# yuxng/PoseCNN

Hardware: NVIDIA H100
Metric: frames/sec on 640x480 RGB, 21 classes, batch 32 (VGG16 + Hough + ROI pose head) (higher is better)
Workload: dtype bf16 operands / fp32 accumulate (conv stack, 1x1 heads), fp16 operands / fp32 accumulate (fc6-fc8), fp32 / int32 elsewhere

## Files before the change

### include/posecnn_b200.h

```cpp
#ifndef POSECNN_B200_H_
#define POSECNN_B200_H_

#include <stddef.h>
#include <stdint.h>

#ifdef __cplusplus
extern "C" {
#endif

#define PCNN_OK 0
#define PCNN_E_INVALID (-1)
#define PCNN_E_WORKSPACE (-2)
#define PCNN_E_CUDA (-3)

#define PCNN_MAX_ROI 128
#define PCNN_HOUGH_MAX_ROWS (PCNN_MAX_ROI * 9)

const char* pcnn_last_error(void);
int pcnn_version(void);

int pcnn_hough_vote_workspace_bytes(int B, int H, int W, int C, int skip_pixels, float threshold_vote,
                                    size_t* bytes);
int pcnn_hough_vote_fwd(const int32_t* label, const float* vertex, const float* extents, const float* meta,
                        const float* gt, int B, int H, int W, int C, int num_gt, int num_meta, int is_train,
                        float inlier_threshold, int label_threshold, float threshold_vote,
                        float threshold_percentage, int skip_pixels, float* top_box, float* top_pose,
                        float* top_target, float* top_weight, int32_t* top_domain, int32_t* num_rois,
                        int32_t* status, void* workspace, size_t workspace_bytes, void* stream);
int pcnn_hough_vote_fwd_ex(const int32_t* label, const float* vertex, const float* lowres, const float* bias_vertex,
                           const float* extents, const float* meta, const float* gt, int B, int batch_global,
                           int batch_offset, int H, int W, int C, int num_gt, int num_meta, int is_train,
                           float inlier_threshold, int label_threshold, float threshold_vote,
                           float threshold_percentage, int skip_pixels, float* top_box, float* top_pose,
                           float* top_target, float* top_weight, int32_t* top_domain, int32_t* num_rois,
                           int32_t* status, void* workspace, size_t workspace_bytes, void* stream);
int pcnn_hough_vote_planes(const int32_t* label, const float* vertex, const float* extents, const float* meta,
                           int B, int H, int W, int C, int num_meta, float inlier_threshold,
                           int label_threshold, int skip_pixels, float* votes, void* workspace,
                           size_t workspace_bytes, void* stream);
int pcnn_hough_vote_bwd(float* grad_label, float* grad_vertex, int B, int H, int W, int C, void* stream);

int pcnn_roi_pool_fwd(const float* bottom, const float* rois, int num_rois, int channel_rois, int batch,
                      int height, int width, int channels, int pooled_height, int pooled_width,
                      float spatial_scale, int pool_channel, float* top, int32_t* argmax, void* stream);
int pcnn_roi_pool_fwd_bf16(const void* bottom_bf16, const float* rois, int num_rois, int channel_rois, int batch,
                           int height, int width, int channels, int pooled_height, int pooled_width,
                           float spatial_scale, float* top, int32_t* argmax, void* stream);
int pcnn_roi_pool_bwd(const float* top_diff, const int32_t* argmax, const float* rois, int batch, int num_rois,
                      int channel_rois, int height, int width, int channels, int pooled_height,
                      int pooled_width, float spatial_scale, int pool_channel, float* bottom_diff,
                      void* stream);

int pcnn_hard_label_fwd(const float* prob, const int32_t* gt, int B, int H, int W, int C, float threshold,
                        float* top, void* stream);
int pcnn_hard_label_bwd(int B, int H, int W, int C, float* grad_prob, float* grad_gt, void* stream);

int pcnn_backproject_fwd(const float* data, const float* label, const float* depth, const float* meta,
                         const float* label_3d, int B, int H, int W, int Cf, int C, int num_meta,
                         int grid_size, int kernel_size, float threshold, float* top_data, float* top_label,
                         float* top_flag, void* stream);
int pcnn_backproject_bwd(const float* top_diff, const float* depth, const float* meta, int B, int H, int W,
                         int Cf, int num_meta, int grid_size, float* bottom_diff, void* stream);

int pcnn_project_fwd(const float* data, const float* depth, const float* meta, int B, int H, int W, int Cf,
                     int num_meta, int grid_size, float* top, void* stream);
int pcnn_project_bwd(const float* top_diff, const float* depth, const float* meta, int B, int H, int W, int Cf,
                     int num_meta, int grid_size, int kernel_size, float threshold, float* bottom_diff,
                     void* stream);

int pcnn_average_distance_workspace_bytes(int N, size_t* bytes);
int pcnn_average_distance_fwd(const float* prediction, const float* target, const float* weight,
                              const float* point, const float* symmetry, int N, int C, int P, float margin,
                              float* loss, float* bottom_diff, void* workspace, size_t workspace_bytes,
                              void* stream);
int pcnn_average_distance_bwd(const float* top_diff, const float* bottom_diff, int N, int channels,
                              float* output, void* stream);

int pcnn_conv_bf16_tc(const void* in_bf16, const void* weights_bf16, const float* bias, void* out_bf16, int B,
                      int H, int W, int Cin, int Cout, int ksize, int relu, int block_n, void* stream);
int pcnn_conv_pool_bf16_tc(const void* in_bf16, const void* weights_bf16, const float* bias, void* out_pooled_bf16,
                           int B, int H, int W, int Cin, int Cout, int ksize, int relu, int block_n, void* stream);
int pcnn_conv3x3_small_cin(const float* in, const float* weights_hwio, const float* bias, void* out_bf16, int B,
                           int H, int W, int Cin, int Cout, int relu, void* stream);
int pcnn_im2col_c3(const void* in, int in_is_u8, const float* mean3_host, void* out_bf16, int B, int H, int W,
                   void* stream);
int pcnn_im2col_depth(const float* depth, const float* mean3_host, void* out_bf16, int B, int H, int W, void* stream);
int pcnn_conv1_fused_tc(const void* in, int in_is_u8, const float* mean3_host, const void* weights_bf16,
                        const float* bias, void* out_bf16, int B, int H, int W, int relu, void* stream);
int pcnn_conv1_depth_fused_tc(const float* depth, const float* mean3_host, const void* weights_bf16, const float* bias,
                              void* out_bf16, int B, int H, int W, int relu, void* stream);
int pcnn_maxpool2x2_bf16(const void* in_bf16, void* out_bf16, int B, int H, int W, int C, void* stream);

int pcnn_conv_wgrad_workspace_bytes(int B, int H, int W, int Cin, int Cout, int ksize, size_t* bytes);
int pcnn_conv_wgrad_bf16_tc(const void* x_bf16, const void* dz_bf16, int B, int H, int W, int Cin, int Cout, int ksize,
                            float scale, const float* w_f32, float decay, float* dW, void* workspace, size_t workspace_bytes,
                            void* stream);
int pcnn_fc_wgrad_f16_tc(const void* x_f16, const void* dy_f16, int rows, int Cin, int Cout, float scale, const float* w_f32,
                         float decay, float* dW, void* workspace, size_t workspace_bytes, void* stream);
int pcnn_bias_ws_bytes(int C, size_t* bytes);
int pcnn_relu_bwd_bf16(const void* g_bf16, const void* y_bf16, size_t npix, int C, int has_relu, void* dz_bf16, float scale,
                       const float* b, float decay, float* db, void* bias_ws, size_t bias_ws_bytes, void* stream);
int pcnn_maxpool_relu_bwd_bf16(const void* g_bf16, const void* y_bf16, int B, int H, int W, int C, void* dz_bf16, float scale,
                               const float* b, float decay, float* db, void* bias_ws, size_t bias_ws_bytes, void* stream);
int pcnn_add_to_bf16(const void* a_bf16, const void* b_bf16, const float* b_f32, size_t n, void* out_bf16, void* stream);

int pcnn_add_up2_bf16(const void* a4_bf16, const void* a5_bf16, int B, int h, int w, int C, void* out_bf16, void* stream);
int pcnn_up2_bwd_bf16(const void* dadd_bf16, const void* y5_bf16, int B, int h, int w, int C, void* d5_bf16, void* stream);
int pcnn_pack_lowres(const void* sc_bf16, int Cs, const void* vt_bf16, int Cv, int B, int h, int w, int C, float* lowres, void* stream);
int pcnn_up8_heads_bwd_ex(const float* prob, const float* score, const int32_t* gt, const float* cls_loss_out, float upstream_cls,
                          float threshold, const float* vertex_pred, const float* lowres, const float* bias_vertex, const float* centers,
                          const float* vertex_loss_out, float upstream_vertex, float w_inside, float sigma, int B, int h, int w, int C,
                          int Cs, int Cv, void* d_sc_bf16, void* d_vt_bf16, float* dbias, void* workspace, size_t workspace_bytes,
                          void* stream);
int pcnn_pose_chain_bwd(const float* bottom_diff, const float* poses_tanh, const float* poses_weight, int N, int D, float upstream,
                        void* dpre_f16, int ld, void* stream);
int pcnn_sgd_momentum(float* w, float* accum, const float* grad, size_t n, float lr, float mu, float wd, float gscale, void* copy16,
                      int kind, void* stream);
int pcnn_loss_cls_hard_raw_fwd(const float* score_raw, const float* prob, const int32_t* gt, int B, int H, int W, int C,
                               float threshold, float* loss_out, void* workspace, size_t workspace_bytes, void* stream);
int pcnn_fc_dgrad_f16_tc(const void* dy_f16, const void* w_in_out_f16, int M, int N, int K, const void* relu_mask_f16, void* out_f16,
                         int ld_out, void* workspace, size_t workspace_bytes, void* stream);
int pcnn_transpose16(const void* in, int rows, int cols, void* out, void* stream);
int pcnn_half_to_float(const void* src_f16, size_t n, float scale, float* dst, void* stream);

int pcnn_roi_pool_pair_f16(const void* f5_bf16, int H5, int W5, const void* f4_bf16, int H4, int W4, int C, int B,
                            int batch_offset, const float* rois, int num_rois, int roi_stride, int pooled_h,
                            int pooled_w, float scale5, float scale4, void* out_f16, void* stream);
int pcnn_fc_workspace_bytes(int M, int N, int K, size_t* bytes);
int pcnn_fc_f16_tc(const void* a_f16, const void* w_f16, const float* bias, int M, int N, int K, int n_valid, int act,
                   void* out_f16, int ld_out, float* out_f32, void* workspace, size_t workspace_bytes, void* stream);

int pcnn_domain_tail(const void* fc9_f16, int rows, int ld, const float* w10, const float* b10, const int32_t* label_domain,
                     float loss_scale, float grad_scale, float* domain_score, float* domain_prob, int32_t* domain_label,
                     float* loss, float* amax, float* dw10, float* db10, float* db9, void* dpre9_f16, void* stream);
int pcnn_domain_grad_merge(const void* a_f16, float scale_a, const void* b_f16, float scale_b, size_t n, float* dst, void* stream);

int pcnn_lowres_heads(const void* score4, const void* score5, const void* vert4, const void* vert5,
                      const float* w_score, const float* w_vertex, int B, int h, int w, int Cs, int Cv, int C,
                      float* lowres, void* stream);
int pcnn_up8_heads(const float* lowres, const float* bias_score, const float* bias_vertex, int B, int h, int w,
                   int C, int32_t* label, float* vertex, float* prob, float* score, void* stream);
int pcnn_deconv_bilinear(const float* in, float* out, int B, int h, int w, int C, int k, int s, void* stream);

int pcnn_nms_pose_fwd(const float* rois, const float* poses_init, const float* poses_pred, const int* num_rois_dev,
                      int num_rows, int capacity, int num_classes, float thresh, int per_image, int32_t* keep,
                      float* out_rois, float* out_poses, int32_t* num_keep, void* stream);

int pcnn_vertex_targets_instances_fwd(const int32_t* label, const int32_t* mask, const float* instances, int B, int H, int W,
                                      int C, int I, float w_inside, float* targets, float* weights, void* stream);
int pcnn_pack_pose_meta_fwd(const float* poses, const int32_t* cls, const float* intrinsics, int B, int I, float im_scale,
                            int flip_x, float* pose_blob, int32_t* num_rows, float* meta, void* stream);
int pcnn_train_loss_workspace_bytes(size_t* bytes);
int pcnn_vertex_targets_fwd(const int32_t* label, const float* centers, int B, int H, int W, int C, float w_inside,
                            float* targets, float* weights, void* stream);
int pcnn_loss_cls_hard_fwd(const float* score, const float* prob, const int32_t* gt, int B, int H, int W, int C,
                           float threshold, float* loss_out, float upstream, float* grad_score, void* workspace,
                           size_t workspace_bytes, void* stream);
int pcnn_smooth_l1_vertex_fwd(const float* pred, const float* targets, const float* weights, size_t n, float sigma,
                              float* loss_out, float upstream, float* grad_pred, void* workspace, size_t workspace_bytes,
                              void* stream);
int pcnn_vertex_loss_fused_fwd(const float* pred, const int32_t* label, const float* centers, int B, int H, int W, int C,
                               float w_inside, float sigma, float* loss_out, float upstream, float* grad_pred,
                               void* workspace, size_t workspace_bytes, void* stream);
int pcnn_vertex_loss_fused_lowres_fwd(const float* lowres, const float* bias_vertex, const int32_t* label, const float* centers, int B,
                                      int H, int W, int C, float w_inside, float sigma, float* loss_out, void* workspace,
                                      size_t workspace_bytes, void* stream);

#define PCNN_AUG_BACKGROUND 0
#define PCNN_AUG_CHROMATIC 1
#define PCNN_AUG_DH 2
#define PCNN_AUG_DL 3
#define PCNN_AUG_DS 4
#define PCNN_AUG_NOISE 5
// ... 15 lines not shown
```

### posecnn_b200/conv.py

```python
from __future__ import annotations

import torch

from ._lib import check, lib, ptr, stream


def hwio_to_tc(weights_hwio: torch.Tensor, dtype=torch.bfloat16) -> torch.Tensor:
    kh, kw, ci, co = weights_hwio.shape
    return weights_hwio.permute(3, 0, 1, 2).reshape(co, kh * kw * ci).to(dtype).contiguous()


def hwio_to_tc_dgrad(weights_hwio: torch.Tensor) -> torch.Tensor:
    kh, kw, ci, co = weights_hwio.shape
    flipped = torch.flip(weights_hwio, dims=(0, 1)).permute(0, 1, 3, 2).contiguous()
    return hwio_to_tc(flipped)


def conv_bf16(x: torch.Tensor, w_tc: torch.Tensor, bias: torch.Tensor, ksize: int, relu: bool, block_n: int = 0,
              out: torch.Tensor | None = None) -> torch.Tensor:
    assert x.is_cuda and x.dtype == torch.bfloat16 and x.is_contiguous() and x.dim() == 4
    assert w_tc.dtype == torch.bfloat16 and w_tc.is_contiguous() and bias.dtype == torch.float32
    B, H, W, Cin = x.shape
    Cout = w_tc.shape[0]
    assert w_tc.shape[1] == ksize * ksize * Cin
    if out is None:
        out = torch.empty((B, H, W, Cout), dtype=torch.bfloat16, device=x.device)
    check(lib().pcnn_conv_bf16_tc(ptr(x), ptr(w_tc), ptr(bias), ptr(out), B, H, W, Cin, Cout, int(ksize), int(bool(relu)),
                                  int(block_n), stream()))
    return out


def conv_pool_bf16(x: torch.Tensor, w_tc: torch.Tensor, bias: torch.Tensor, ksize: int, relu: bool, block_n: int = 0) -> torch.Tensor:
    assert x.is_cuda and x.dtype == torch.bfloat16 and x.is_contiguous() and x.dim() == 4
    B, H, W, Cin = x.shape
    Cout = w_tc.shape[0]
    out = torch.empty((B, H // 2, W // 2, Cout), dtype=torch.bfloat16, device=x.device)
    check(lib().pcnn_conv_pool_bf16_tc(ptr(x), ptr(w_tc), ptr(bias), ptr(out), B, H, W, Cin, Cout, int(ksize), int(bool(relu)),
                                       int(block_n), stream()))
    return out


def conv3x3_small_cin(x: torch.Tensor, w_hwio: torch.Tensor, bias: torch.Tensor, relu: bool = True) -> torch.Tensor:
    assert x.is_cuda and x.dtype == torch.float32 and x.is_contiguous()
    B, H, W, Cin = x.shape
    Cout = w_hwio.shape[3]
    out = torch.empty((B, H, W, Cout), dtype=torch.bfloat16, device=x.device)
    check(lib().pcnn_conv3x3_small_cin(ptr(x), ptr(w_hwio.contiguous()), ptr(bias), ptr(out), B, H, W, Cin, Cout,
                                       int(bool(relu)), stream()))
    return out


def maxpool2x2(x: torch.Tensor) -> torch.Tensor:
    assert x.is_cuda and x.dtype == torch.bfloat16 and x.is_contiguous()
    B, H, W, C = x.shape
    out = torch.empty((B, H // 2, W // 2, C), dtype=torch.bfloat16, device=x.device)
    check(lib().pcnn_maxpool2x2_bf16(ptr(x), ptr(out), B, H, W, C, stream()))
    return out


def im2col_c3(x: torch.Tensor, mean=None) -> torch.Tensor:
    import ctypes
    assert x.is_cuda and x.is_contiguous() and x.shape[3] == 3 and x.dtype in (torch.float32, torch.uint8)
    B, H, W, _ = x.shape
    out = torch.empty((B, H, W, 64), dtype=torch.bfloat16, device=x.device)
    m = (ctypes.c_float * 3)(*(mean if mean is not None else (0.0, 0.0, 0.0)))
    check(lib().pcnn_im2col_c3(ptr(x), int(x.dtype == torch.uint8), m, ptr(out), B, H, W, stream()))
    return out


def im2col_depth(depth: torch.Tensor, mean) -> torch.Tensor:
    import ctypes
    assert depth.is_cuda and depth.is_contiguous() and depth.dtype == torch.float32 and depth.dim() == 3
    B, H, W = depth.shape
    out = torch.empty((B, H, W, 64), dtype=torch.bfloat16, device=depth.device)
    m = (ctypes.c_float * 3)(*mean)
    check(lib().pcnn_im2col_depth(ptr(depth), m, ptr(out), B, H, W, stream()))
    return out


def conv1_1_weights_to_tc(w_hwio: torch.Tensor) -> torch.Tensor:
    co = w_hwio.shape[3]
    w = torch.zeros((co, 64), dtype=torch.float32, device=w_hwio.device)
    w[:, :27] = w_hwio.reshape(27, co).t()
    return w.to(torch.bfloat16).contiguous()


def conv1_fused(x: torch.Tensor, w_tc64: torch.Tensor, bias: torch.Tensor, mean=None, relu: bool = True) -> torch.Tensor:
    import ctypes
    assert x.is_cuda and x.is_contiguous() and x.shape[3] == 3 and x.dtype in (torch.float32, torch.uint8)
    assert w_tc64.shape == (64, 64) and w_tc64.dtype == torch.bfloat16
    B, H, W, _ = x.shape
    out = torch.empty((B, H, W, 64), dtype=torch.bfloat16, device=x.device)
    m = (ctypes.c_float * 3)(*(mean if mean is not None else (0.0, 0.0, 0.0)))
    check(lib().pcnn_conv1_fused_tc(ptr(x), int(x.dtype == torch.uint8), m, ptr(w_tc64), ptr(bias), ptr(out), B, H, W,
                                    int(bool(relu)), stream()))
    return out


def conv1_depth_fused(depth: torch.Tensor, w_tc64: torch.Tensor, bias: torch.Tensor, mean, relu: bool = True) -> torch.Tensor:
    import ctypes
    assert depth.is_cuda and depth.is_contiguous() and depth.dtype == torch.float32 and depth.dim() == 3
    B, H, W = depth.shape
    out = torch.empty((B, H, W, 64), dtype=torch.bfloat16, device=depth.device)
    m = (ctypes.c_float * 3)(*mean)
    check(lib().pcnn_conv1_depth_fused_tc(ptr(depth), m, ptr(w_tc64), ptr(bias), ptr(out), B, H, W, int(bool(relu)), stream()))
    return out
```

### posecnn_b200/csrc/conv_tc.cu

```cuda
#include <cuda.h>
#include <cuda_bf16.h>

#include <type_traits>

#include "common.cuh"
#include "tc_common.cuh"

namespace pcnn {
namespace convtc {

constexpr int kTileH = 8, kTileW = 16;
static_assert(kTileH * kTileW == kTileM, "pixel tile = two wgmma M blocks");
constexpr int kABytes = kTileM * kKC * 2;
constexpr int kConsumers = 256;
constexpr int kProducerWarp = kConsumers / 32;
constexpr int kThreadsConv = kConsumers + 128;
constexpr int kConsumerRegs = 232, kProducerRegs = 40;
constexpr int kThreadsRow = kConsumers + 32;
constexpr int kStageBytes = 16 * 1024;

struct ConvParams {
    int B, H, W, Cin, Cout;
    int taps, ksize;
    int tiles_h, tiles_w, n_tiles_n, total_tiles;
// ... 535 lines not shown
                uint32_t pk[4];
#pragma unroll
                for (int q = 0; q < 4; q++) {
                    __nv_bfloat162 b2 = __floats2bfloat162_rn(v[j * 8 + q * 2], v[j * 8 + q * 2 + 1]);
                    pk[q] = *reinterpret_cast<uint32_t*>(&b2);
                }
                *reinterpret_cast<uint4*>(sa + ((j ^ (r & 7)) << 4)) = make_uint4(pk[0], pk[1], pk[2], pk[3]);
            }
            fence_proxy_async();
            __syncwarp();
            if (lane == 0) mbar_arrive(&full[stage]);
        }
    } else {
        const int eg = warp >> 2, wq = warp & 3;
        const bool issuer = (threadIdx.x & 127) == 0;
        if (warp == 0) {
            if (elect_one()) {
                mbar_arrive_expect_tx(wbar, 64 * 128);
                tma_load_2d(sb, &map_w, wbar, 0, 0);
            }
            __syncwarp();
            mbar_wait(wbar, 0);
            for (int n = lane; n < BN; n += 32) {
                const float bv = p.bias[n];
                const __nv_bfloat16 hi = __float2bfloat16_rn(bv);
                const __nv_bfloat16 lo = __float2bfloat16_rn(bv - __bfloat162float(hi));
                uint8_t* rowp = sb + n * 128 + ((3 ^ (n & 7)) << 4);
                *reinterpret_cast<__nv_bfloat16*>(rowp + 6) = hi;
                *reinterpret_cast<__nv_bfloat16*>(rowp + 8) = lo;
            }
            fence_proxy_async();
        }
        asm volatile("bar.sync 7, 256;" ::: "memory");
        const uint64_t db = make_desc(smem_u32(sb));
        uint8_t* my_stage = out_stage + eg * 2 * kStageBytes;
        const __nv_bfloat162 floor2 = __floats2bfloat162_rn(p.relu ? 0.f : -INFINITY, p.relu ? 0.f : -INFINITY);
        int it = 0, obuf = 0;
        for (int tile = blockIdx.x; tile < p.total_tiles; tile += gridDim.x, it++) {
            if ((it & 1) != eg) continue;
            const int tw = tile % p.tiles_w;
            const int rest = tile / p.tiles_w;
            const int th = rest % p.tiles_h, img = rest / p.tiles_h;
            const int stage = it % kC1Stages;
            mbar_wait(&full[stage], (it / kC1Stages) & 1);
            if (issuer) tma_store_wait_read<1>();
            if (eg == 0) asm volatile("bar.sync 1, 128;" ::: "memory");
            else asm volatile("bar.sync 2, 128;" ::: "memory");
            uint8_t* ob = my_stage + obuf * kStageBytes;
            const uint32_t sa = smem_u32(smem + stage * kABytes);
#pragma unroll
            for (int half = 0; half < 2; half++) {
                float acc[BN / 2];
                acc_fence<BN / 2>(acc);
                wgmma_fence();
                const uint64_t da = make_desc(sa + half * 64 * 128);
                wgmma<BN, 0, 0, 0>(acc, da, db, 0);
                wgmma<BN, 0, 0, 0>(acc, da + 2, db + 2, 1);
                wgmma_commit();
                wgmma_wait<0>();
                acc_fence<BN / 2>(acc);
                if (half == 1) release(&empty[stage], lane);
                const int q = lane & 3;
#pragma unroll
                for (int i = 0; i < 2; i++) {
                    const int r = half * 64 + wq * 16 + (lane >> 2) + 8 * i;
#pragma unroll
                    for (int jj = 0; jj < 8; jj++) {
                        uint32_t pk = pack_bf16(acc[4 * jj + 2 * i], acc[4 * jj + 2 * i + 1]);
                        __nv_bfloat162 b2 = __hmax2(*reinterpret_cast<__nv_bfloat162*>(&pk), floor2);
                        *reinterpret_cast<__nv_bfloat162*>(ob + r * 128 + ((jj ^ (r & 7)) << 4) + 4 * q) = b2;
                    }
                }
            }
            fence_proxy_async();
            if (eg == 0) asm volatile("bar.sync 1, 128;" ::: "memory");
            else asm volatile("bar.sync 2, 128;" ::: "memory");
            if (issuer) {
                tma_store_4d(&map_out, ob, 0, tw * kTileW, th * kTileH, img);
                tma_store_commit();
            }
            obuf ^= 1;
        }
        if (issuer) tma_store_wait_all();
    }
}

template <int CO_PER_THREAD>
__global__ void __launch_bounds__(256)
k_conv_small_cin(const float* __restrict__ in, const float* __restrict__ w ,
                 const float* __restrict__ bias, __nv_bfloat16* __restrict__ out, int B, int H, int W, int Cin, int Cout,
                 int relu)
{
    extern __shared__ float sw[];
    const int K = 9 * Cin;
    for (int i = threadIdx.x; i < K * Cout; i += blockDim.x) sw[i] = w[i];
    for (int i = threadIdx.x; i < Cout; i += blockDim.x) sw[K * Cout + i] = bias[i];
    __syncthreads();
    const int groups = Cout / CO_PER_THREAD;
    const size_t total = (size_t)B * H * W * groups;
    for (size_t idx = (size_t)blockIdx.x * blockDim.x + threadIdx.x; idx < total; idx += (size_t)gridDim.x * blockDim.x) {
        const int g = (int)(idx % groups);
        const size_t pix = idx / groups;
        const int x = (int)(pix % W), y = (int)((pix / W) % H);
        const size_t n = pix / ((size_t)W * H);
        float acc[CO_PER_THREAD];
#pragma unroll
        for (int k = 0; k < CO_PER_THREAD; k++) acc[k] = sw[K * Cout + g * CO_PER_THREAD + k];
        for (int r = 0; r < 3; r++) {
            const int yy = y + r - 1;
            if (yy < 0 || yy >= H) continue;
            for (int s = 0; s < 3; s++) {
                const int xx = x + s - 1;
                if (xx < 0 || xx >= W) continue;
                const float* ip = in + ((n * H + yy) * W + xx) * Cin;
                for (int c = 0; c < Cin; c++) {
                    const float v = __ldg(ip + c);
                    const float* wp = sw + ((r * 3 + s) * Cin + c) * Cout + g * CO_PER_THREAD;
#pragma unroll
                    for (int k = 0; k < CO_PER_THREAD; k++) acc[k] = fmaf(v, wp[k], acc[k]);
                }
            }
        }
        __nv_bfloat16* op = out + pix * Cout + g * CO_PER_THREAD;
#pragma unroll
        for (int k = 0; k < CO_PER_THREAD; k += 2) {
            float v0 = acc[k], v1 = acc[k + 1];
            if (relu) { v0 = fmaxf(v0, 0.f); v1 = fmaxf(v1, 0.f); }
            *reinterpret_cast<__nv_bfloat162*>(op + k) = __floats2bfloat162_rn(v0, v1);
        }
    }
}

template <typename TIn>
__global__ void __launch_bounds__(256)
k_im2col_c3(const TIn* __restrict__ in, __nv_bfloat16* __restrict__ out, int H, int W, float m0, float m1, float m2)
{
    constexpr int kSeg = 128;
    constexpr int kInCh = std::is_same<TIn, DepthIn>::value ? 1 : 3;
    __shared__ float patch[3][(kSeg + 2) * 3];
    const int y = blockIdx.y, n = blockIdx.z, x0 = blockIdx.x * kSeg, t = threadIdx.x;
    const TIn* img = in + (size_t)n * H * W * kInCh;
    constexpr int kRow = (kSeg + 2) * 3;
    for (int i = t; i < 3 * kRow; i += 256) {
        const int r = i / kRow, rem = i - r * kRow, px = rem / 3, c = rem - px * 3;
        const int yy = y + r - 1, xx = x0 + px - 1;
        float v = 0.f;
        if (yy >= 0 && yy < H && xx >= 0 && xx < W) {
            if constexpr (std::is_same<TIn, DepthIn>::value)
                v = __fsub_rn(depth_gray(img[yy * W + xx].d), c == 0 ? m0 : (c == 1 ? m1 : m2));
            else
                v = (float)img[(yy * W + xx) * 3 + c] - (c == 0 ? m0 : (c == 1 ? m1 : m2));
        }
        patch[r][rem] = v;
    }
    __syncthreads();
    const int j = t & 7;
#pragma unroll
    for (int pass = 0; pass < kSeg / 32; pass++) {
        const int xl = pass * 32 + (t >> 3), x = x0 + xl;
        if (x >= W) break;
        __align__(16) __nv_bfloat16 v[8];
#pragma unroll
        for (int e = 0; e < 8; e++) {
            const int k = j * 8 + e;
            float val = 0.f;
            if (k < 27) {
// ... 179 lines not shown
    PCNN_REQUIRE(H % 2 == 0 && W % 2 == 0 && C % 8 == 0, "maxpool: needs even H, W and C %% 8 == 0 (got %d,%d,%d)", H, W, C);
    size_t total = (size_t)B * (H / 2) * (W / 2) * (C / 8);
    int blocks = (int)((total + 255) / 256 < (size_t)kNumSMs * 16 ? (total + 255) / 256 : (size_t)kNumSMs * 16);
    k_maxpool2x2_bf16<<<blocks, 256, 0, (cudaStream_t)stream>>>((const __nv_bfloat16*)in, (__nv_bfloat16*)out, B, H, W, C);
    return check_launch("maxpool2x2");
}

extern "C" int pcnn_im2col_c3(const void* in, int in_is_u8, const float* mean3_host, void* out_bf16, int B, int H, int W,
                              void* stream)
{
    PCNN_REQUIRE(in && out_bf16, "im2col: NULL tensor pointer");
    float m0 = 0.f, m1 = 0.f, m2 = 0.f;
    if (mean3_host) { m0 = mean3_host[0]; m1 = mean3_host[1]; m2 = mean3_host[2]; }
    PCNN_REQUIRE(H <= 65535 && B <= 65535, "im2col: image too tall for the launch grid");
    dim3 grid((W + 127) / 128, H, B);
    cudaStream_t st = (cudaStream_t)stream;
    if (in_is_u8)
        k_im2col_c3<unsigned char><<<grid, 256, 0, st>>>((const unsigned char*)in, (__nv_bfloat16*)out_bf16, H, W, m0, m1, m2);
    else
        k_im2col_c3<float><<<grid, 256, 0, st>>>((const float*)in, (__nv_bfloat16*)out_bf16, H, W, m0, m1, m2);
    return check_launch("im2col_c3");
}

extern "C" int pcnn_im2col_depth(const float* depth, const float* mean3_host, void* out_bf16, int B, int H, int W, void* stream)
{
    PCNN_REQUIRE(depth && out_bf16, "im2col_depth: NULL tensor pointer");
    PCNN_REQUIRE(B >= 1 && H >= 1 && W >= 1, "im2col_depth: bad shape (%d,%d,%d)", B, H, W);
    PCNN_REQUIRE(H <= 65535 && B <= 65535, "im2col_depth: image too tall for the launch grid");
    float m0 = 0.f, m1 = 0.f, m2 = 0.f;
    if (mean3_host) { m0 = mean3_host[0]; m1 = mean3_host[1]; m2 = mean3_host[2]; }
    dim3 grid((W + 127) / 128, H, B);
    k_im2col_c3<DepthIn><<<grid, 256, 0, (cudaStream_t)stream>>>((const DepthIn*)depth, (__nv_bfloat16*)out_bf16, H, W, m0, m1, m2);
    return check_launch("im2col_depth");
}

static int conv1_fused_impl(const void* in, int in_kind, const float* mean3_host, const void* weights_bf16,
                            const float* bias, void* out_bf16, int B, int H, int W, int relu, void* stream);

extern "C" int pcnn_conv1_fused_tc(const void* in, int in_is_u8, const float* mean3_host, const void* weights_bf16,
                                   const float* bias, void* out_bf16, int B, int H, int W, int relu, void* stream)
{
    return conv1_fused_impl(in, in_is_u8 ? 1 : 0, mean3_host, weights_bf16, bias, out_bf16, B, H, W, relu, stream);
}

extern "C" int pcnn_conv1_depth_fused_tc(const float* depth, const float* mean3_host, const void* weights_bf16,
                                         const float* bias, void* out_bf16, int B, int H, int W, int relu, void* stream)
{
    return conv1_fused_impl(depth, 2, mean3_host, weights_bf16, bias, out_bf16, B, H, W, relu, stream);
}

static int conv1_fused_impl(const void* in, int in_kind, const float* mean3_host, const void* weights_bf16,
                                   const float* bias, void* out_bf16, int B, int H, int W, int relu, void* stream)
{
    PCNN_REQUIRE(in && weights_bf16 && bias && out_bf16, "conv1: NULL tensor pointer");
    PCNN_REQUIRE(B >= 1 && H >= 1 && W >= 1, "conv1: bad shape");
    float m0 = 0.f, m1 = 0.f, m2 = 0.f;
    if (mean3_host) { m0 = mean3_host[0]; m1 = mean3_host[1]; m2 = mean3_host[2]; }
    CUtensorMap mw, mo;
    int rc = make_map_weights(&mw, weights_bf16, 64, 64, 64);
    if (rc) return rc;
    rc = make_map_nhwc(&mo, out_bf16, B, H, W, 64, 64);
    if (rc) return rc;
    ConvParams p;
    p.B = B; p.H = H; p.W = W; p.Cin = 3; p.Cout = 64; p.ksize = 3; p.taps = 9;
    p.tile_h = kTileH; p.tile_w = kTileW;
    p.tiles_h = (H + kTileH - 1) / kTileH;
    p.tiles_w = (W + kTileW - 1) / kTileW;
    p.n_tiles_n = 1;
    p.total_tiles = B * p.tiles_h * p.tiles_w;
    p.relu = relu; p.pool = 0; p.bias = bias; p.kc_outer = 0;
    int dev = 0, sms = kNumSMs;
    cudaGetDevice(&dev);
    cudaDeviceGetAttribute(&sms, cudaDevAttrMultiProcessorCount, dev);
    int grid = p.total_tiles < sms ? p.total_tiles : sms;
    cudaStream_t st = (cudaStream_t)stream;
    PCNN_SMEM_OPTIN(k_conv1_tc<unsigned char>, kC1Smem, "conv1_tc<u8>");
    PCNN_SMEM_OPTIN(k_conv1_tc<float>, kC1Smem, "conv1_tc<f32>");
    PCNN_SMEM_OPTIN(k_conv1_tc<DepthIn>, kC1Smem, "conv1_tc<depth>");
    if (in_kind == 1) k_conv1_tc<unsigned char><<<grid, kC1Threads, kC1Smem, st>>>((const unsigned char*)in, mw, mo, p, m0, m1, m2);
    else if (in_kind == 2) k_conv1_tc<DepthIn><<<grid, kC1Threads, kC1Smem, st>>>((const DepthIn*)in, mw, mo, p, m0, m1, m2);
    else k_conv1_tc<float><<<grid, kC1Threads, kC1Smem, st>>>((const float*)in, mw, mo, p, m0, m1, m2);
    return check_launch("conv1_fused_tc");
}
```

### posecnn_b200/networks/vgg16_convs.py

```python
from __future__ import annotations

import math

import numpy as np
import torch

from .. import conv, pose_head
from .._lib import check, lib, ptr, stream
from ..hough_voting_gpu_layer import hough_voting_gpu_op
from ..roi_pooling_layer import roi_pooling_op
from ..utils import nms as dev_nms

PIXEL_MEANS = (102.9801, 115.9465, 122.7717)

VGG_CFG = [("conv1_1", 3, 64), ("conv1_2", 64, 64), "pool1", ("conv2_1", 64, 128), ("conv2_2", 128, 128), "pool2",
           ("conv3_1", 128, 256), ("conv3_2", 256, 256), ("conv3_3", 256, 256), "pool3", ("conv4_1", 256, 512),
           ("conv4_2", 512, 512), ("conv4_3", 512, 512), "pool4", ("conv5_1", 512, 512), ("conv5_2", 512, 512),
           ("conv5_3", 512, 512)]


class vgg16_convs:
    def __init__(self, input_format="COLOR", num_classes=22, num_units=64, scales=(1.0,), threshold_label=1.0,
                 vote_threshold=-1.0, vertex_reg_2d=True, vertex_reg_3d=False, pose_reg=True, adaptation=False,
                 trainable=True, is_train=False, device="cuda", fold_vertex_head=True):
# ... 41 lines not shown
            shapes["domain_score/weights"] = (256, 2); shapes["domain_score/biases"] = (2,)
        return shapes

    def init_random(self, seed=0, bias_std=0.0):
        g = torch.Generator(device="cpu").manual_seed(seed)
        for name, shp in self.param_shapes().items():
            if name.endswith("weights"):
                fan_in = int(np.prod(shp[:-1]))
                t = torch.randn(shp, generator=g) * math.sqrt(2.0 / fan_in)
            else:
                t = torch.randn(shp, generator=g) * bias_std if bias_std > 0 else torch.zeros(shp)
            self.params[name] = t.to(self.device)
        self.prepare()
        return self

    def calibrate_background(self, data, meta_data, extents, background_fraction=0.75, **forward_kwargs):
        self.forward(data, meta_data, extents, want_prob=False, sync_rois=False, **forward_kwargs)
        C = self.num_classes
        B, H, W, _ = data.shape
        lab = torch.empty((B, H, W), dtype=torch.int32, device=data.device)
        vert = torch.empty((B, H, W, 3 * C), dtype=torch.float32, device=data.device)
        lowres = self._last_lowres
        bias = self.params["score/biases"]
        base = float(bias[0])

        def fg_fraction(b0):
            bias[0] = b0
            check(lib().pcnn_up8_heads(ptr(lowres), ptr(bias), ptr(self.params["vertex_pred/biases"]), B, H // 8, W // 8, C,
                                       ptr(lab), ptr(vert), ptr(None), ptr(None), stream()))
            return float((lab > 0).float().mean())

        scale = float(lowres[..., :C].abs().max()) + 1.0
        lo, hi = base - scale, base + scale
        for _ in range(24):
            mid = 0.5 * (lo + hi)
            if fg_fraction(mid) > 1.0 - background_fraction:
                lo = mid
            else:
                hi = mid
        bias[0] = hi
        return hi - base

    def load(self, data_dict: dict):
        for k, v in data_dict.items():
            if isinstance(v, dict):
                for kk, vv in v.items():
                    self.params[f"{k}/{kk}"] = torch.as_tensor(np.asarray(vv), dtype=torch.float32, device=self.device)
                    if self.input_format == "RGBD" and k.startswith("conv") and "score" not in k:
                        self.params[f"{k}_p/{kk}"] = self.params[f"{k}/{kk}"].clone()
            else:
                self.params[k] = torch.as_tensor(np.asarray(v), dtype=torch.float32, device=self.device)
        self.prepare()
        return self

    def prepare(self):
        P, T = self.params, self._tc
        T.clear()
        for name, shp in self.param_shapes().items():
            if not name.endswith("weights") or name.startswith("fc") or name in ("score/weights", "vertex_pred/weights", "domain_score/weights"):
                continue
            w = P[name]
            if w.shape[2] == 3:
                T[name] = conv.conv1_1_weights_to_tc(w)
            else:
                T[name] = conv.hwio_to_tc(w)
        for name in ("fc6", "fc7", "fc8"):
            T[f"{name}/weights"] = pose_head.fc_weights_to_tc(P[f"{name}/weights"])
        if self.domain_branch:
            T["fc9/weights"] = pose_head.fc_weights_to_tc(P["fc9/weights"])
            T["domain_score/w"] = P["domain_score/weights"].t().contiguous()
        T["score/w"] = P["score/weights"].reshape(self.num_units, self.num_classes).contiguous()
        T["vertex_pred/w"] = P["vertex_pred/weights"].reshape(128, 3 * self.num_classes).contiguous()
        if self.fold_vertex_head:
            Wp = T["vertex_pred/w"].double()
            for name in ("score_conv4_vertex", "score_conv5_vertex"):
                w = P[f"{name}/weights"].reshape(-1, 128).double() @ Wp
                b = P[f"{name}/biases"].double() @ Wp
                wpad = torch.zeros((1, 1, w.shape[0], 128), dtype=torch.float32, device=w.device)
                wpad[0, 0, :, :w.shape[1]] = w.float()
                bpad = torch.zeros((128,), dtype=torch.float32, device=w.device)
                bpad[:b.shape[0]] = b.float()
                T[f"{name}/folded_weights"], T[f"{name}/folded_biases"] = conv.hwio_to_tc(wpad), bpad

    def _trunk(self, data, sfx=""):
        P, T = self.params, self._tc
        if data.dim() == 3:
            x = conv.conv1_depth_fused(data, T[f"conv1_1{sfx}/weights"], P[f"conv1_1{sfx}/biases"], PIXEL_MEANS, True)
        else:
            mean = PIXEL_MEANS if data.dtype == torch.uint8 else None
            x = conv.conv1_fused(data, T[f"conv1_1{sfx}/weights"], P[f"conv1_1{sfx}/biases"], mean, True)
        feats = {}
        cfg = VGG_CFG[1:]
        i = 0
        while i < len(cfg):
            item = cfg[i]
            if isinstance(item, str):
                x = conv.maxpool2x2(x)
                i += 1
                continue
            name = item[0]
            fuse_pool = i + 1 < len(cfg) and isinstance(cfg[i + 1], str) and name not in ("conv4_3", "conv5_3")
            if fuse_pool:
                x = conv.conv_pool_bf16(x, T[f"{name}{sfx}/weights"], P[f"{name}{sfx}/biases"], 3, True)
                i += 2
                continue
            x = conv.conv_bf16(x, T[f"{name}{sfx}/weights"], P[f"{name}{sfx}/biases"], 3, True)
            if name in ("conv4_3", "conv5_3"):
                feats[name] = x
            i += 1
        return feats

    def forward(self, data, meta_data, extents, poses=None, data_p=None, want_prob=False, sync_rois=True, want_score=False,
                dense_vertex=True, batch_global=None, batch_offset=0, depth=None):
        C = self.num_classes
        L = self.layers = {}
        P, T = self.params, self._tc
        B, H, W, _ = data.shape
        assert H % 16 == 0 and W % 16 == 0, "pad the image to a multiple of 16 (lib/utils/blob.py:48-58)"
        f = self._trunk(data)
        c4, c5 = f["conv4_3"], f["conv5_3"]
        L["conv4_3"], L["conv5_3"] = c4, c5
        if self.input_format == "RGBD":
            fp = self._trunk(depth if depth is not None else data_p, "_p")
            h4, h5 = torch.cat([c4, fp["conv4_3"]], 3), torch.cat([c5, fp["conv5_3"]], 3)
        else:
            h4, h5 = c4, c5
        s5 = conv.conv_bf16(h5, T["score_conv5/weights"], P["score_conv5/biases"], 1, True)
        s4 = conv.conv_bf16(h4, T["score_conv4/weights"], P["score_conv4/biases"], 1, True)
        L["score_conv4"], L["score_conv5"] = s4, s5
        if self.fold_vertex_head:
            v5 = conv.conv_bf16(c5, T["score_conv5_vertex/folded_weights"], T["score_conv5_vertex/folded_biases"], 1, False)
            v4 = conv.conv_bf16(c4, T["score_conv4_vertex/folded_weights"], T["score_conv4_vertex/folded_biases"], 1, False)
            w_vertex = None
        else:
            v5 = conv.conv_bf16(c5, T["score_conv5_vertex/weights"], P["score_conv5_vertex/biases"], 1, False)
            v4 = conv.conv_bf16(c4, T["score_conv4_vertex/weights"], P["score_conv4_vertex/biases"], 1, False)
            L["score_conv4_vertex"], L["score_conv5_vertex"] = v4, v5
            w_vertex = T["vertex_pred/w"]
        h, w = H // 8, W // 8
        lowres = torch.empty((B, h, w, 4 * C), dtype=torch.float32, device=data.device)
        check(lib().pcnn_lowres_heads(ptr(s4), ptr(s5), ptr(v4), ptr(v5), ptr(T["score/w"]), ptr(w_vertex), B, h, w,
                                      self.num_units, 128, C, ptr(lowres), stream()))
        self._last_lowres = lowres
        label = torch.empty((B, H, W), dtype=torch.int32, device=data.device)
        vertex = torch.empty((B, H, W, 3 * C), dtype=torch.float32, device=data.device) if dense_vertex else None
        prob = torch.empty((B, H, W, C), dtype=torch.float32, device=data.device) if want_prob else None
        score = torch.empty((B, H, W, C), dtype=torch.float32, device=data.device) if want_score else None
        check(lib().pcnn_up8_heads(ptr(lowres), ptr(P["score/biases"]), ptr(P["vertex_pred/biases"]), B, h, w, C, ptr(label),
                                   ptr(vertex), ptr(prob), ptr(score), stream()))
        L["label_2d"] = label
        if dense_vertex:
            L["vertex_pred"] = vertex
        if want_prob:
            L["prob_normalized"] = prob
        if want_score:
            L["score"] = score
        if not self.vertex_reg_2d:
            return L
        Bg = B if batch_global is None else int(batch_global)
        box, pose, target, weight, domain, num_rois, status = hough_voting_gpu_op.hough_voting_gpu_capacity(
            label, vertex, extents, meta_data, poses, self.is_train, self.vote_threshold, self.vote_percentage, self.skip_pixels,
            lowres=lowres, bias_vertex=P["vertex_pred/biases"], batch_global=Bg, batch_offset=batch_offset)
        cap_rows = max(1, min(box.shape[0], (128 // Bg) * B * (9 if self.is_train else 1)))
        rois = box[:cap_rows]
        L["rois_capacity"], L["num_rois"] = rois, num_rois
        L["hough_status"] = status
        L["poses_init"], L["poses_target"], L["poses_weight"] = pose[:cap_rows], target[:cap_rows], weight[:cap_rows]
        if self.pose_reg:
            if self.is_train:
                rl = rois if not batch_offset else torch.cat([rois[:, :1] - float(batch_offset), rois[:, 1:]], 1)
                p5, a5 = roi_pooling_op.roi_pool(c5, rl, 7, 7, 1.0 / 16.0, 0)
                p4, a4 = roi_pooling_op.roi_pool(c4, rl, 7, 7, 1.0 / 8.0, 0)
                L["pool5_argmax"], L["pool4_argmax"] = a5, a4
                x = (p5 + p4).reshape(cap_rows, -1).clamp(-65504.0, 65504.0).to(torch.float16)
            else:
                x = pose_head.roi_pool_pair(c5, c4, rois, 7, 7, 1.0 / 16.0, 1.0 / 8.0, batch_offset)
# ... 105 lines not shown
```

Measured before the change: 2939.

## Fuse conv1_1, conv1_2 and pool1 into one warp-specialized persistent kernel

```diff
diff --git a/include/posecnn_b200.h b/include/posecnn_b200.h
--- a/include/posecnn_b200.h
+++ b/include/posecnn_b200.h
@@ -89,6 +89,9 @@
                         const float* bias, void* out_bf16, int B, int H, int W, int relu, void* stream);
 int pcnn_conv1_depth_fused_tc(const float* depth, const float* mean3_host, const void* weights_bf16, const float* bias,
                               void* out_bf16, int B, int H, int W, int relu, void* stream);
+int pcnn_conv1_block_tc(const void* in, int in_kind, const float* mean3_host, const void* w1_bf16, const float* b1,
+                        const void* w2_bf16, const float* b2, void* out_pooled_bf16, int B, int H, int W, int relu, int grid,
+                        void* stream);
 int pcnn_maxpool2x2_bf16(const void* in_bf16, void* out_bf16, int B, int H, int W, int C, void* stream);
 
 int pcnn_conv_wgrad_workspace_bytes(int B, int H, int W, int Cin, int Cout, int ksize, size_t* bytes);
diff --git a/posecnn_b200/conv.py b/posecnn_b200/conv.py
--- a/posecnn_b200/conv.py
+++ b/posecnn_b200/conv.py
@@ -105,3 +105,27 @@
     m = (ctypes.c_float * 3)(*mean)
     check(lib().pcnn_conv1_depth_fused_tc(ptr(depth), m, ptr(w_tc64), ptr(bias), ptr(out), B, H, W, int(bool(relu)), stream()))
     return out
+
+
+def conv1_block_ok(H: int, W: int) -> bool:
+    return H % 2 == 0 and W % 2 == 0 and W >= 128
+
+
+def conv1_block(x: torch.Tensor, w1_tc64: torch.Tensor, b1: torch.Tensor, w2_tc: torch.Tensor, b2: torch.Tensor, mean=None,
+                relu: bool = True, grid: int = 0) -> torch.Tensor:
+    import ctypes
+    assert x.is_cuda and x.is_contiguous()
+    if x.dim() == 3:
+        assert x.dtype == torch.float32 and mean is not None
+        kind = 2
+    else:
+        assert x.dim() == 4 and x.shape[3] == 3 and x.dtype in (torch.float32, torch.uint8)
+        kind = 1 if x.dtype == torch.uint8 else 0
+    assert w1_tc64.shape == (64, 64) and w1_tc64.dtype == torch.bfloat16
+    assert w2_tc.shape == (64, 576) and w2_tc.dtype == torch.bfloat16 and w2_tc.is_contiguous()
+    B, H, W = x.shape[:3]
+    out = torch.empty((B, H // 2, W // 2, 64), dtype=torch.bfloat16, device=x.device)
+    m = (ctypes.c_float * 3)(*(mean if mean is not None else (0.0, 0.0, 0.0)))
+    check(lib().pcnn_conv1_block_tc(ptr(x), kind, m, ptr(w1_tc64), ptr(b1), ptr(w2_tc), ptr(b2), ptr(out), B, H, W,
+                                    int(bool(relu)), int(grid), stream()))
+    return out
diff --git a/posecnn_b200/csrc/conv_tc.cu b/posecnn_b200/csrc/conv_tc.cu
--- a/posecnn_b200/csrc/conv_tc.cu
+++ b/posecnn_b200/csrc/conv_tc.cu
@@ -641,6 +641,313 @@
             obuf ^= 1;
         }
         if (issuer) tma_store_wait_all();
+    }
+}
+
+constexpr int kB1Slots = 6;
+constexpr int kB1SlotBytes = 17 * 1024;
+constexpr int kB1InPx = kRowPx + 4;
+constexpr int kB1InRow = kB1InPx * 3;
+constexpr int kB1Px = 2 * kPatchW;
+constexpr int kB1Blocks = (kB1Px + 63) / 64;
+constexpr int kB1ABytes = (kB1Blocks + 1) / 2 * 64 * 128;
+constexpr int kB1Threads = kConsumers + 128;
+constexpr int kB1Conv2Regs = 128, kB1Conv1Regs = 232;
+constexpr int kB1W2Off = kB1Slots * kB1SlotBytes;
+constexpr int kB1W1Off = kB1W2Off + 9 * 64 * 128;
+constexpr int kB1AOff = kB1W1Off + 64 * 128;
+constexpr int kB1OutOff = kB1AOff + kB1ABytes;
+constexpr int kB1InOff = kB1OutOff + kStageBytes;
+constexpr int kB1BarOff = kB1InOff + 4 * kB1InRow * 2;
+constexpr int kB1Smem = kB1BarOff + 256 + 1024;
+static_assert(kB1Smem <= 232448, "conv1_block: shared memory above the sm_90 opt-in limit");
+
+struct Block1Params {
+    int B, H, W;
+    int tiles_h, tiles_w, items;
+    int relu;
+    const float* bias1;
+    const float* bias2;
+};
+
+constexpr int kB1Loads = (4 * kB1InRow + 127) / 128;
+
+template <typename TIn>
+struct Conv1Loader {
+    using Raw = typename std::conditional<sizeof(TIn) == 1, uint32_t, float>::type;
+    Raw raw[kB1Loads];
+
+    __device__ __forceinline__ static bool at(int idx, int ya, int x0, int H, int W, int& yy, int& xx, int& ch)
+    {
+        const int ir = idx / kB1InRow, rem = idx - ir * kB1InRow, pc = rem / 3;
+        ch = rem - pc * 3;
+        yy = ya - 1 + ir;
+        xx = x0 - 2 + pc;
+        return idx < 4 * kB1InRow && yy >= 0 && yy < H && xx >= 0 && xx < W;
+    }
+    __device__ __forceinline__ void load(const TIn* base, int ya, int x0, int H, int W, int t)
+    {
+#pragma unroll
+        for (int i = 0; i < kB1Loads; i++) {
+            int yy, xx, ch;
+            at(t + 128 * i, ya, x0, H, W, yy, xx, ch);
+            yy = min(max(yy, 0), H - 1);
+            xx = min(max(xx, 0), W - 1);
+            if constexpr (std::is_same<TIn, DepthIn>::value) raw[i] = __ldg(&base[(size_t)yy * W + xx].d);
+            else raw[i] = __ldg(base + ((size_t)yy * W + xx) * 3 + ch);
+        }
+    }
+    __device__ __forceinline__ void stage(__nv_bfloat16* s, int ya, int x0, int H, int W, int t, float m0, float m1, float m2) const
+    {
+#pragma unroll
+        for (int i = 0; i < kB1Loads; i++) {
+            const int idx = t + 128 * i;
+            int yy, xx, ch;
+            const bool ok = at(idx, ya, x0, H, W, yy, xx, ch);
+            const float m = ch == 0 ? m0 : (ch == 1 ? m1 : m2);
+            float v = 0.f;
+            if constexpr (std::is_same<TIn, DepthIn>::value) { if (ok) v = __fsub_rn(depth_gray(raw[i]), m); }
+            else { if (ok) v = (float)raw[i] - m; }
+            if (idx < 4 * kB1InRow) s[idx] = __float2bfloat16_rn(v);
+        }
+    }
+};
+
+template <typename TIn>
+__global__ void __launch_bounds__(kB1Threads, 1)
+k_conv1_block(const TIn* __restrict__ in, const __grid_constant__ CUtensorMap map_w1, const __grid_constant__ CUtensorMap map_w2,
+              const __grid_constant__ CUtensorMap map_out , const Block1Params p,
+              float m0, float m1, float m2)
+{
+    extern __shared__ uint8_t smem_raw[];
+    uint8_t* smem = reinterpret_cast<uint8_t*>((reinterpret_cast<uintptr_t>(smem_raw) + 1023) & ~(uintptr_t)1023);
+    uint8_t* sW2 = smem + kB1W2Off;
+    uint8_t* sW1 = smem + kB1W1Off;
+    uint8_t* sA = smem + kB1AOff;
+    uint8_t* out_stage = smem + kB1OutOff;
+    __nv_bfloat16* sIn = reinterpret_cast<__nv_bfloat16*>(smem + kB1InOff);
+    uint64_t* rfull = reinterpret_cast<uint64_t*>(smem + kB1BarOff);
+    uint64_t* rempty = rfull + kB1Slots;
+    uint64_t* w1bar = rempty + kB1Slots;
+    uint64_t* w2bar = w1bar + 1;
+    const int warp = threadIdx.x >> 5, lane = threadIdx.x & 31;
+    const int lo = (int)((long long)blockIdx.x * p.items / gridDim.x);
+    const int hi = (int)((long long)(blockIdx.x + 1) * p.items / gridDim.x);
+
+    if (threadIdx.x == kConsumers) {
+        asm volatile("prefetch.tensormap [%0];" ::"l"(&map_w1) : "memory");
+        asm volatile("prefetch.tensormap [%0];" ::"l"(&map_w2) : "memory");
+        asm volatile("prefetch.tensormap [%0];" ::"l"(&map_out) : "memory");
+        for (int s = 0; s < kB1Slots; s++) { mbar_init(&rfull[s], 4); mbar_init(&rempty[s], kConsumers / 32); }
+        mbar_init(w1bar, 1);
+        mbar_init(w2bar, 1);
+        fence_barrier_init();
+    }
+    __syncthreads();
+    if (threadIdx.x == kConsumers) {
+        mbar_arrive_expect_tx(w1bar, 64 * 128);
+        tma_load_2d(sW1, &map_w1, w1bar, 0, 0);
+        mbar_arrive_expect_tx(w2bar, 9 * 64 * 128);
+        for (int tap = 0; tap < 9; tap++) tma_load_2d(sW2 + tap * 64 * 128, &map_w2, w2bar, tap * 64, 0);
+    }
+
+    if (warp >= kConsumers / 32) {
+        setmaxnreg_inc<kB1Conv1Regs>();
+        const int t = threadIdx.x - kConsumers, wq = warp - kConsumers / 32;
+        if (wq == 0) {
+            mbar_wait(w1bar, 0);
+            for (int n = lane; n < 64; n += 32) {
+                const float bv = p.bias1[n];
+                const __nv_bfloat16 bh = __float2bfloat16_rn(bv);
+                const __nv_bfloat16 bl = __float2bfloat16_rn(bv - __bfloat162float(bh));
+                uint8_t* rowp = sW1 + n * 128 + ((3 ^ (n & 7)) << 4);
+                *reinterpret_cast<__nv_bfloat16*>(rowp + 6) = bh;
+                *reinterpret_cast<__nv_bfloat16*>(rowp + 8) = bl;
+            }
+            fence_proxy_async();
+        }
+        asm volatile("bar.sync 2, 128;" ::: "memory");
+        constexpr int kInCh = std::is_same<TIn, DepthIn>::value ? 1 : 3;
+        const uint64_t db = make_desc(smem_u32(sW1));
+        const uint32_t a_u32 = smem_u32(sA);
+        const __nv_bfloat162 floor2 = __floats2bfloat162_rn(p.relu ? 0.f : -INFINITY, p.relu ? 0.f : -INFINITY);
+        const uint16_t* sIn16 = reinterpret_cast<const uint16_t*>(sIn);
+        Conv1Loader<TIn> ld;
+        int item = lo, u = 0;
+        auto pair_of = [&](int it, int uu, int& ya, int& x0, const TIn*& base) {
+            const int yp = it % p.tiles_h, rest = it / p.tiles_h;
+            ya = 2 * yp - 1 + 2 * uu;
+            x0 = (rest % p.tiles_w) * kRowPx;
+            base = in + (size_t)(rest / p.tiles_w) * p.H * p.W * kInCh;
+        };
+        int ya, x0;
+        const TIn* base;
+        if (item < hi) {
+            pair_of(item, u, ya, x0, base);
+            ld.load(base, ya, x0, p.H, p.W, t);
+        }
+        uint32_t seq = 0;
+        while (item < hi) {
+            {
+                ld.stage(sIn, ya, x0, p.H, p.W, t, m0, m1, m2);
+                int nitem = item, nu = u + 1;
+                if (nu == 2) { nitem++; nu = nitem % p.tiles_h == 0 ? 0 : 1; }
+                int nya = 0, nx0 = 0;
+                const TIn* nbase = in;
+                if (nitem < hi) {
+                    pair_of(nitem, nu, nya, nx0, nbase);
+                    ld.load(nbase, nya, nx0, p.H, p.W, t);
+                }
+                const int s0 = seq % kB1Slots, s1 = (seq + 1) % kB1Slots;
+                asm volatile("bar.sync 2, 128;" ::: "memory");
+#pragma unroll
+                for (int pass = 0; pass < 3; pass++) {
+                    const int q = pass * 128 + t;
+                    if (q < kB1Px) {
+                        const int rr = q >= kPatchW, c = q - rr * kPatchW;
+                        uint16_t v[32];
+#pragma unroll
+                        for (int dy = 0; dy < 3; dy++)
+#pragma unroll
+                            for (int k = 0; k < 9; k++) v[dy * 9 + k] = sIn16[(rr + dy) * kB1InRow + 3 * c + k];
+                        v[27] = 0x3f80; v[28] = 0x3f80; v[29] = 0; v[30] = 0; v[31] = 0;
+                        const int b = q >> 6, ar = (b >> 1) * 64 + (q & 63);
+                        uint8_t* sa = sA + ar * 128;
+#pragma unroll
+                        for (int j = 0; j < 4; j++) {
+                            uint32_t pk[4];
+#pragma unroll
+                            for (int e = 0; e < 4; e++) pk[e] = (uint32_t)v[8 * j + 2 * e] | ((uint32_t)v[8 * j + 2 * e + 1] << 16);
+                            *reinterpret_cast<uint4*>(sa + (((j + 4 * (b & 1)) ^ (ar & 7)) << 4)) = make_uint4(pk[0], pk[1], pk[2], pk[3]);
+                        }
+                    }
+                }
+                fence_proxy_async();
+                asm volatile("bar.sync 2, 128;" ::: "memory");
+                float acc[kB1Blocks][32];
+#pragma unroll
+                for (int b = 0; b < kB1Blocks; b++) acc_fence<32>(acc[b]);
+                wgmma_fence();
+#pragma unroll
+                for (int b = 0; b < kB1Blocks; b++) {
+                    const uint64_t da = make_desc(a_u32 + (b >> 1) * 64 * 128 + (b & 1) * 64);
+                    wgmma<64, 0, 0, 0>(acc[b], da, db, 0);
+                    wgmma<64, 0, 0, 0>(acc[b], da + 2, db + 2, 1);
+                }
+                wgmma_commit();
+                wgmma_wait<0>();
+#pragma unroll
+                for (int b = 0; b < kB1Blocks; b++) acc_fence<32>(acc[b]);
+                mbar_wait(&rempty[s0], ((seq / kB1Slots) & 1) ^ 1);
+                mbar_wait(&rempty[s1], (((seq + 1) / kB1Slots) & 1) ^ 1);
+                const int q4 = lane & 3;
+#pragma unroll
+                for (int b = 0; b < kB1Blocks; b++) {
+#pragma unroll
+                    for (int i = 0; i < 2; i++) {
+                        const int q = b * 64 + wq * 16 + (lane >> 2) + 8 * i;
+                        if (q >= kB1Px) continue;
+                        const int rr = q >= kPatchW, c = q - rr * kPatchW;
+                        const int y = ya + rr, x = x0 - 1 + c;
+                        const bool inside = y >= 0 && y < p.H && x >= 0 && x < p.W;
+                        uint8_t* dst = smem + (rr ? s1 : s0) * kB1SlotBytes + c * 128;
+#pragma unroll
+                        for (int jj = 0; jj < 8; jj++) {
+                            uint32_t pk = pack_bf16(acc[b][4 * jj + 2 * i], acc[b][4 * jj + 2 * i + 1]);
+                            __nv_bfloat162 b2 = __hmax2(*reinterpret_cast<__nv_bfloat162*>(&pk), floor2);
+                            uint32_t o = inside ? *reinterpret_cast<uint32_t*>(&b2) : 0u;
+                            *reinterpret_cast<uint32_t*>(dst + ((jj ^ (c & 7)) << 4) + 4 * q4) = o;
+                        }
+                    }
+                }
+                fence_proxy_async();
+                __syncwarp();
+                if (lane == 0) { mbar_arrive(&rfull[s0]); mbar_arrive(&rfull[s1]); }
+                seq += 2;
+                item = nitem; u = nu; ya = nya; x0 = nx0; base = nbase;
+            }
+        }
+    } else {
+        setmaxnreg_dec<kB1Conv2Regs>();
+        constexpr int kH = 32;
+        const int wg = warp >> 2, wq = warp & 3;
+        const int row = wg * 64 + wq * 16 + (lane >> 2);
+        const uint32_t ring_u32 = smem_u32(smem) + wg * 64 * 128;
+        float acc[2 * kH];
+        int obuf = 0;
+        uint32_t seq = 0;
+        mbar_wait(w2bar, 0);
+        for (int item = lo; item < hi; item++) {
+            const int yp = item % p.tiles_h;
+            const int rest = item / p.tiles_h;
+            const int tw = rest % p.tiles_w, img = rest / p.tiles_w;
+            const int y0 = 2 * yp, x0 = tw * kRowPx;
+            const bool restart = item == lo || yp == 0;
+            const uint32_t first = restart ? seq : seq - 2;
+            seq += restart ? 4 : 2;
+            uint32_t slot[4];
+#pragma unroll
+            for (int rho = 0; rho < 4; rho++) {
+                const uint32_t s = first + rho;
+                mbar_wait(&rfull[s % kB1Slots], (s / kB1Slots) & 1);
+                slot[rho] = ring_u32 + (s % kB1Slots) * kB1SlotBytes;
+            }
+            acc_fence<2 * kH>(acc);
+            wgmma_fence();
+#pragma unroll
+            for (int o = 0; o < 4; o++) {
+                const int rho = o == 0 ? 1 : (o == 1 ? 2 : (o == 2 ? 0 : 3));
+#pragma unroll
+                for (int s3 = 0; s3 < 3; s3++) {
+                    const uint64_t da = make_desc(slot[rho] + (uint32_t)(s3 * 128));
+#pragma unroll
+                    for (int j = 0; j < 2; j++) {
+                        const int r = rho - j;
+                        if (r < 0 || r > 2) continue;
+                        const uint64_t db = make_desc(smem_u32(sW2 + (r * 3 + s3) * 64 * 128));
+#pragma unroll
+                        for (int k = 0; k < kKC / 16; k++)
+                            wgmma<64, 0, 0, 0>(acc + j * kH, da + (uint64_t)(k * 2), db + (uint64_t)(k * 2), (o | s3 | k) != 0);
+                    }
+                }
+            }
+            wgmma_commit();
+            wgmma_wait<0>();
+            acc_fence<2 * kH>(acc);
+            const bool keep = item + 1 < hi && (item + 1) % p.tiles_h != 0;
+#pragma unroll
+            for (int rho = 0; rho < 4; rho++)
+                if (rho < 2 || !keep) release(&rempty[(first + rho) % kB1Slots], lane);
+            if (threadIdx.x == 0) tma_store_wait_read<1>();
+            consumer_sync();
+            uint8_t* ob = out_stage + obuf * (kStageBytes / 2);
+            const int q = lane & 3;
+#pragma unroll
+            for (int i = 0; i < 2; i++) {
+                const int r = row + 8 * i;
+                const int prow = r >> 1;
+#pragma unroll
+                for (int jj = 0; jj < 8; jj++) {
+                    const int c = 8 * jj + 2 * q;
+                    float v0 = fmaxf(acc[4 * jj + 2 * i], acc[kH + 4 * jj + 2 * i]) + __ldg(p.bias2 + c);
+                    float v1 = fmaxf(acc[4 * jj + 2 * i + 1], acc[kH + 4 * jj + 2 * i + 1]) + __ldg(p.bias2 + c + 1);
+                    if (p.relu) { v0 = fmaxf(v0, 0.f); v1 = fmaxf(v1, 0.f); }
+                    uint32_t pk = pack_bf16(v0, v1);
+                    uint32_t o1 = __shfl_xor_sync(0xffffffffu, pk, 4);
+                    __nv_bfloat162 m2 = __hmax2(*reinterpret_cast<__nv_bfloat162*>(&pk), *reinterpret_cast<__nv_bfloat162*>(&o1));
+                    if ((lane & 4) == 0)
+                        *reinterpret_cast<__nv_bfloat162*>(ob + prow * 128 + ((jj ^ (prow & 7)) << 4) + 4 * q) = m2;
+                }
+            }
+            fence_proxy_async();
+            consumer_sync();
+            if (threadIdx.x == 0) {
+                tma_store_4d(&map_out, ob, 0, x0 >> 1, y0 >> 1, img);
+                tma_store_commit();
+            }
+            obuf ^= 1;
+        }
+        if (threadIdx.x == 0) tma_store_wait_all();
     }
 }
 
@@ -986,3 +1293,45 @@
     else k_conv1_tc<float><<<grid, kC1Threads, kC1Smem, st>>>((const float*)in, mw, mo, p, m0, m1, m2);
     return check_launch("conv1_fused_tc");
 }
+
+extern "C" int pcnn_conv1_block_tc(const void* in, int in_kind, const float* mean3_host, const void* w1_bf16, const float* b1,
+                                   const void* w2_bf16, const float* b2, void* out_pooled, int B, int H, int W, int relu,
+                                   int grid, void* stream)
+{
+    PCNN_REQUIRE(in && w1_bf16 && b1 && w2_bf16 && b2 && out_pooled, "conv1_block: NULL tensor pointer");
+    PCNN_REQUIRE(in_kind >= 0 && in_kind <= 2, "conv1_block: in_kind must be 0 (f32), 1 (u8) or 2 (depth), got %d", in_kind);
+    PCNN_REQUIRE(B >= 1 && H >= 2 && H % 2 == 0 && W >= kRowPx && W % 2 == 0,
+                 "conv1_block: needs even H >= 2 and even W >= %d (got %d x %d)", kRowPx, H, W);
+    float m0 = 0.f, m1 = 0.f, m2 = 0.f;
+    if (mean3_host) { m0 = mean3_host[0]; m1 = mean3_host[1]; m2 = mean3_host[2]; }
+    CUtensorMap mw1, mw2, mo;
+    int rc = make_map_weights(&mw1, w1_bf16, 64, 64, 64);
+    if (rc) return rc;
+    rc = make_map_weights(&mw2, w2_bf16, 9 * 64, 64, 64);
+    if (rc) return rc;
+    rc = make_map_nhwc(&mo, out_pooled, B, H / 2, W / 2, 64, 64, kRowPx / 2, 1);
+    if (rc) return rc;
+    Block1Params p;
+    p.B = B; p.H = H; p.W = W;
+    p.tiles_h = H / 2;
+    p.tiles_w = (W + kRowPx - 1) / kRowPx;
+    p.items = B * p.tiles_h * p.tiles_w;
+    p.relu = relu; p.bias1 = b1; p.bias2 = b2;
+    int dev = 0, sms = kNumSMs;
+    cudaGetDevice(&dev);
+    cudaDeviceGetAttribute(&sms, cudaDevAttrMultiProcessorCount, dev);
+    int g = grid > 0 && grid < sms ? grid : sms;
+    if (g > p.items) g = p.items;
+    cudaStream_t st = (cudaStream_t)stream;
+    if (in_kind == 1) {
+        PCNN_SMEM_OPTIN(k_conv1_block<unsigned char>, kB1Smem, "conv1_block<u8>");
+        k_conv1_block<unsigned char><<<g, kB1Threads, kB1Smem, st>>>((const unsigned char*)in, mw1, mw2, mo, p, m0, m1, m2);
+    } else if (in_kind == 2) {
+        PCNN_SMEM_OPTIN(k_conv1_block<DepthIn>, kB1Smem, "conv1_block<depth>");
+        k_conv1_block<DepthIn><<<g, kB1Threads, kB1Smem, st>>>((const DepthIn*)in, mw1, mw2, mo, p, m0, m1, m2);
+    } else {
+        PCNN_SMEM_OPTIN(k_conv1_block<float>, kB1Smem, "conv1_block<f32>");
+        k_conv1_block<float><<<g, kB1Threads, kB1Smem, st>>>((const float*)in, mw1, mw2, mo, p, m0, m1, m2);
+    }
+    return check_launch("conv1_block_tc");
+}
diff --git a/posecnn_b200/networks/vgg16_convs.py b/posecnn_b200/networks/vgg16_convs.py
--- a/posecnn_b200/networks/vgg16_convs.py
+++ b/posecnn_b200/networks/vgg16_convs.py
@@ -147,16 +147,21 @@
                 bpad[:b.shape[0]] = b.float()
                 T[f"{name}/folded_weights"], T[f"{name}/folded_biases"] = conv.hwio_to_tc(wpad), bpad
 
-    def _trunk(self, data, sfx=""):
+    def _trunk(self, data, sfx="", fuse_conv1=True):
         P, T = self.params, self._tc
-        if data.dim() == 3:
-            x = conv.conv1_depth_fused(data, T[f"conv1_1{sfx}/weights"], P[f"conv1_1{sfx}/biases"], PIXEL_MEANS, True)
+        depth = data.dim() == 3
+        mean = PIXEL_MEANS if depth or data.dtype == torch.uint8 else None
+        w1, b1 = T[f"conv1_1{sfx}/weights"], P[f"conv1_1{sfx}/biases"]
+        i = 0
+        if fuse_conv1 and conv.conv1_block_ok(data.shape[1], data.shape[2]):
+            x = conv.conv1_block(data, w1, b1, T[f"conv1_2{sfx}/weights"], P[f"conv1_2{sfx}/biases"], mean, True)
+            i = 2
+        elif depth:
+            x = conv.conv1_depth_fused(data, w1, b1, mean, True)
         else:
-            mean = PIXEL_MEANS if data.dtype == torch.uint8 else None
-            x = conv.conv1_fused(data, T[f"conv1_1{sfx}/weights"], P[f"conv1_1{sfx}/biases"], mean, True)
+            x = conv.conv1_fused(data, w1, b1, mean, True)
         feats = {}
         cfg = VGG_CFG[1:]
-        i = 0
         while i < len(cfg):
             item = cfg[i]
             if isinstance(item, str):
```

Result: no change. 2947, median of 6 (+0.3%).
